# adam-kerrigan/pybader

Measured on AMD Instinct MI355X. Metric: Mvoxels/s neargrid assign+refine on 512^3 grid, higher is better.
Workload: dtype f64; 1 GPU; 512^3 synthetic 8-Gaussian-atom cubic cell (BASELINE config 3), neargrid assign + neargrid edge refinement changed:2, density resident in HBM; method=neargrid, device_driven_slab_step=False, basins=8

## Files before the change

include/bader_hip.h:

```cpp
#ifndef BADER_HIP_H
#define BADER_HIP_H

#include <stdint.h>

#ifdef __cplusplus
extern "C" {
#endif

typedef struct xb_ctx xb_ctx;

enum { XB_OK = 0, XB_E_ARG = -1, XB_E_HIP = -2, XB_E_STATE = -3, XB_E_LIMIT = -4, XB_E_COMM = -5,
       XB_E_SHORT = -6  };

enum { XB_I8 = 1, XB_I16 = 2, XB_I32 = 4, XB_I64 = 8 };

enum { XB_METHOD_ONGRID = 0, XB_METHOD_NEARGRID = 1 };
enum { XB_REFINE_ALL = 0, XB_REFINE_CHANGED = 1 };

const char *xb_last_error(void);
int xb_device_count(void);
int xb_create(int device, xb_ctx **out);
void xb_destroy(xb_ctx *c);
int xb_sync(xb_ctx *c);
void *xb_stream(xb_ctx *c);
// ... 188 lines not shown
enum {
    XB_REGIONS_BOXES = 1,
    XB_REGIONS_BRICKS = 2
};
enum { XB_DROP_TABLE_AND_MAXIMA = 2 };
enum {
    XB_CHECK_NO_MIRROR = 1,
    XB_CHECK_GENERIC_WALKER = 2,
    XB_CHECK_FULL_TGRAD = 4,
    XB_CHECK_LIST_DILATE = 8,
    XB_CHECK_WIDE_HALO = 16,
    XB_CHECK_NO_EC_SHARE = 32,
    XB_CHECK_IO_GATHER = 64
};
#define XB_CHECK_BRICK_LOOKUP 128
enum {
    XB_DBG_EC_PASSES = 4,
    XB_DBG_SLAB_STATS = 16,
    XB_DBG_STAGE_WAIT = 32,
    XB_DBG_SHORT_TIERS = 64
};
int xb_set_option(xb_ctx *c, int key, int value);
int xb_host_alloc(int64_t bytes, void **out);
int xb_host_free(void *p);
int xb_memory_stats(xb_ctx *c, int64_t *bytes_total, int64_t *bytes_table, int64_t *bytes_scratch);
int xb_box_stats(xb_ctx *c, int64_t *n_boxes, int64_t *box_voxels);
int xb_brick_labels(xb_ctx *c, int32_t *out, int64_t capacity, int64_t dims[3]);
int xb_slow_path_stats(xb_ctx *c, int64_t *assign_total, int64_t *refine_total);
int xb_deferred_stats(xb_ctx *c, int64_t *refine_total);
int xb_growth_stats(xb_ctx *c, int64_t *retries, int64_t *kill_launches);

int xb_comm_unique_id(uint8_t id_out[128]);
int xb_comm_init(xb_ctx *c, int rank, int nranks, const uint8_t id_in[128]);
int xb_comm_destroy(xb_ctx *c);
int xb_comm_exchange_planes(xb_ctx *c, int which, int n_send, const int32_t *send_peer, const int64_t *send_xa,
                            const int64_t *send_xb, int n_recv, const int32_t *recv_peer, const int64_t *recv_xa,
                            const int64_t *recv_xb);
int xb_comm_allreduce_i64(xb_ctx *c, int64_t *inout, int64_t n, int op);
int xb_comm_allgather_i64(xb_ctx *c, const int64_t *in, int64_t n, int64_t *out);
int xb_comm_share_brick_masks(xb_ctx *c, const int64_t *first, const int64_t *count);
int xb_comm_allgather_block(xb_ctx *c, int which, const int64_t *first, const int64_t *count);
int xb_comm_allreduce_block(xb_ctx *c);
int xb_comm_info(xb_ctx *c, int64_t out[4]);
int xb_comm_stats(xb_ctx *c, int64_t *bytes_sent);
// ... 6 lines not shown
```

pybader_amd/_lib.py:

```python
import ctypes as C
import threading
import os

import numpy as np

HERE = os.path.dirname(os.path.abspath(__file__))
LIB_PATH = os.environ.get('XB_LIBRARY') or os.path.join(HERE, 'libbader_hip.so')

METHODS = {'ongrid': 0, 'neargrid': 1}
REFINE_MODES = {'all': 0, 'changed': 1}
DTYPE_CODE = {np.dtype(np.int8): 1, np.dtype(np.int16): 2, np.dtype(np.int32): 4, np.dtype(np.int64): 8}
(XB_XC_EDGES, XB_XC_CHANGED, XB_XC_ESCAPED, XB_XC_TRAVELLING, XB_XC_SLOW, XB_XC_LOST, XB_XC_MINE, XB_XC_ROUNDS,
 XB_XC_COUNT) = range(9)
(XB_TIMER_ASSIGN, XB_TIMER_OG_MASKS, XB_TIMER_EDGE_FIND, XB_TIMER_REFINE_TRACE, XB_TIMER_MASKS_GROWTH, XB_TIMER_BRICK_MASKS,
 XB_TIMER_TRACE, XB_TIMER_BRICK_RECORDS, XB_TIMER_MOMENTS, XB_TIMER_ADJACENCY, XB_TIMER_MERGE, XB_TIMER_COUNT) = range(12)
XB_OPT_REGIONS = 1
XB_REGIONS_BOXES, XB_REGIONS_BRICKS = 1, 2
XB_OPT_CROSS_CHECK = 2
(XB_CHECK_NO_MIRROR, XB_CHECK_GENERIC_WALKER, XB_CHECK_FULL_TGRAD, XB_CHECK_LIST_DILATE, XB_CHECK_WIDE_HALO,
 XB_CHECK_NO_EC_SHARE, XB_CHECK_IO_GATHER) = (1, 2, 4, 8, 16, 32, 64)
CROSS_CHECK_BRICK_LOOKUP = 128
XB_OPT_DEBUG = 3
XB_DBG_EC_PASSES, XB_DBG_SLAB_STATS, XB_DBG_STAGE_WAIT, XB_DBG_SHORT_TIERS = 4, 16, 32, 64
XB_OPT_EC_GROUPS = 4
XB_OPT_EC_QCAP = 5
XB_OPT_DROP_TABLE = 6
XB_DROP_TABLE_AND_MAXIMA = 2
XB_OPT_KILL_LAUNCHES = 17
XB_OPT_SELF_EXCHANGE = 19
XB_OPT_ASYNC_COMM = 24
XB_OPT_WEIGHT_NO_LABELS = 30
XB_VORONOI_FULL_SEARCH = 1
XB_VORONOI_CAND_MAX = 512
XB_CRITICAL_FLOOD = 1
(XB_CRITICAL_MAXIMA, XB_CRITICAL_BOND_VOXELS, XB_CRITICAL_BOND_SUM, XB_CRITICAL_RING_VOXELS, XB_CRITICAL_RING_SUM,
 XB_CRITICAL_MINIMA, XB_CRITICAL_COUNTS) = range(7)
# ... 108 lines not shown
    'xb_plane_elems': (_i64, [_vp]),
    'xb_copy_planes': (_int, [_vp, _int, _int, _vp, _i64, _i64]),
    'xb_label_wire': (_int, [_vp, _int, _vp]),
    'xb_host_alloc': (_int, [_i64, _vp]),
    'xb_host_free': (_int, [_vp]),
    'xb_brick_masks_copy': (_int, [_vp, _int, _vp, _i64, _i64]),
    'xb_set_halo': (_int, [_vp, _i64]),
    'xb_kernel_time': (_int, [_vp, _int, _pdbl, _pi64]),
    'xb_kernel_time_reset': (_int, [_vp]),
    'xb_enable_timing': (_int, [_vp, _int]),
    'xb_set_option': (_int, [_vp, _int, _int]),
    'xb_box_stats': (_int, [_vp, _pi64, _pi64]),
    'xb_brick_labels': (_int, [_vp, _vp, _i64, _pi64]),
    'xb_slow_path_stats': (_int, [_vp, _pi64, _pi64]),
    'xb_deferred_stats': (_int, [_vp, _pi64]),
    'xb_growth_stats': (_int, [_vp, _pi64, _pi64]),
    'xb_comm_unique_id': (_int, [_vp]),
    'xb_comm_init': (_int, [_vp, _int, _int, _vp]),
    'xb_comm_destroy': (_int, [_vp]),
    'xb_comm_exchange_planes': (_int, [_vp, _int, _int, _vp, _pi64, _pi64, _int, _vp, _pi64, _pi64]),
    'xb_comm_allreduce_i64': (_int, [_vp, _pi64, C.c_int64, _int]),
    'xb_comm_allgather_i64': (_int, [_vp, _pi64, C.c_int64, _pi64]),
    'xb_comm_share_brick_masks': (_int, [_vp, _pi64, _pi64]),
    'xb_comm_allgather_block': (_int, [_vp, _int, _pi64, _pi64]),
    'xb_comm_allreduce_block': (_int, [_vp]),
    'xb_slab_supported': (_int, [_vp, _int, _pi64]),
    'xb_slab_assign_masks': (_int, [_vp, _int, _int]),
    'xb_slab_assign_trace': (_int, [_vp]),
    'xb_slab_assign_finish': (_int, [_vp, _pi64, _pi64]),
    'xb_slab_refine_pass': (_int, [_vp]),
# ... 906 lines not shown
    def slow_path_stats(self):
        a, b = C.c_int64(), C.c_int64()
        check(self.lib.xb_slow_path_stats(self.h, C.byref(a), C.byref(b)))
        return a.value, b.value

    def growth_stats(self):
        a, b = C.c_int64(), C.c_int64()
        check(self.lib.xb_growth_stats(self.h, C.byref(a), C.byref(b)))
        return a.value, b.value

    def deferred_stats(self):
        a = C.c_int64()
        check(self.lib.xb_deferred_stats(self.h, C.byref(a)))
        return a.value

    def sync(self):
        check(self.lib.xb_sync(self.h))


def critical_lut():
    out = np.zeros(XB_CRITICAL_LUT_SIZE, np.uint8)
    check(load().xb_critical_lut(_ptr(out)))
    return out


def hirshfeld_images(lattice, atoms_cart, species, r_cut):
    lat, at = _f64(lattice).reshape(9), _f64(atoms_cart).reshape(-1, 3)
    sp, rc = np.ascontiguousarray(species, dtype=np.int32).reshape(-1), _f64(r_cut).reshape(-1)
    if sp.shape[0] != at.shape[0]:
        raise ValueError(f'hirshfeld_images: {sp.shape[0]} species for {at.shape[0]} atoms')
# ... 36 lines not shown
```

pybader_amd/csrc/bader_hip.hip:

```cpp
#include "bader_kernels.h"
#include "../../include/bader_hip.h"

#include <algorithm>
#include <cmath>
#include <cstdarg>
#include <cstdio>
#include <cstring>
#include <mutex>
#include <string>
#include <thread>
#include <vector>

static thread_local long long xb_waits = 0;
static inline hipError_t xb_counted_sync(hipStream_t s) { xb_waits++; return (hipStreamSynchronize)(s); }
#define hipStreamSynchronize(s) xb_counted_sync(s)

#include "k_common.h"
#include "k_masks.h"
#include "k_fused.h"
#include "k_trace.h"
#include "k_ongrid.h"
#include "k_edges.h"
#include "k_sums.h"
#include "k_text.h"
// ... 49 lines not shown
    long long ec_buf_cap = 0;
    double *dist_dev = nullptr;
    int *boxbuf = nullptr;
    int *box_max_tab = nullptr;
    int n_boxes = 0;
    long long box_voxels = 0;
    struct Options {
        int boxes = 1, bricks = 1;
        int mirror = 1;
        int lean = 1;
        int mask_diag = 1;
        int tile_dilate = 1;
        int narrow_halo = 1;
        int ec_share = 1;
        int nb_bits = 1;
        int io_tiled = 1;
        int dbg = 0;
        int ec_groups = 256;
        int ec_qcap = EC_Q;
        int self_exchange = 0;
        int async_comm = 0;
        bool weight_no_labels = false;
    } opt;
    int *ec_share = nullptr;
    std::vector<int64_t> esc_starts, esc_offsets, esc_vox;
    unsigned long long *ec_pend = nullptr;
    int8_t *ec_pflag = nullptr;
    std::vector<int8_t> esc_complete;
    bool has_vacuum = true;
    bool vac_by_tol = false;
// ... 7 lines not shown
    int *walk = nullptr;
    int table_margin = -1;
    bool table_prebuilt = false;
    int table_stage = 0;
    std::vector<int> window_seeds;
    bool window_ties = true;
    bool slab_sparse = false;
    int ec_local_n = 0;
    int walk_n_out = 0;
    void *walk_out_dev = nullptr;
    std::vector<int64_t> walk_host, res_host;
    int walk_n_res = 0;
    void *walk_in = nullptr, *walk_out2 = nullptr, *walk_res = nullptr;
    long long walk_cap = 0;
    long long stat_deferred = 0;
    long long stat_ovf_assign = 0, stat_ovf_refine = 0;
    int *bres_last = nullptr;
    int *blab = nullptr;
    int nbk[3] = {0, 0, 0};
    bool grad_valid = false;
    bool grad_nb = false;
    bool brick_max_valid = false;
    int grad_cover = 0;
    unsigned char *brick_rec = nullptr;
    unsigned long long *nb_tab = nullptr;
    void *xbuf = nullptr;
    int slab_rank = 0, slab_nranks = 0, slab_stage = 0;
    void *wbuf[2] = {nullptr, nullptr};
    void *wk_in = nullptr;
    int wbuf_ranks = 0, walk_last = -1, walk_round = 0, wcap = 0;
    int walk_send = 0;
    int grow_kill_launches = 6;
    long long stat_grow_retries = 0;
    bool defer_wait = false;
    bool pending_assign = false;
    int64_t pending_n_maxima = 0;
    int grad_rule = 0;
// ... 180 lines not shown
#include "host_weight.h"
#include "host_moments.h"
#include "host_adjacency.h"
#include "host_merge.h"
#include "host_voronoi.h"
#include "host_critical.h"
#include "host_stencil.h"
#include "host_hirshfeld.h"

int xb_set_option(xb_ctx *c, int key, int value) {
    if (!c) return fail(XB_E_ARG, "null ctx");
    bool ok = true;
    switch (key) {
    case XB_OPT_REGIONS: c->opt.boxes = (value & XB_REGIONS_BOXES) != 0; c->opt.bricks = (value & XB_REGIONS_BRICKS) != 0; break;
    case XB_OPT_CROSS_CHECK:
        if (!(ok = value >= 0 && value < 2 * XB_CHECK_BRICK_LOOKUP)) break;
        c->opt.mirror = !(value & XB_CHECK_NO_MIRROR);
        c->opt.lean = !(value & XB_CHECK_GENERIC_WALKER);
        c->opt.mask_diag = !(value & XB_CHECK_FULL_TGRAD);
        c->opt.tile_dilate = !(value & XB_CHECK_LIST_DILATE);
        c->opt.narrow_halo = !(value & XB_CHECK_WIDE_HALO);
        c->opt.ec_share = !(value & XB_CHECK_NO_EC_SHARE);
        c->opt.io_tiled = !(value & XB_CHECK_IO_GATHER);
        c->opt.nb_bits = !(value & XB_CHECK_BRICK_LOOKUP);
        break;
    case XB_OPT_DEBUG: c->opt.dbg = value; break;
    case XB_OPT_EC_GROUPS: if ((ok = value >= 1 && value <= 4096)) c->opt.ec_groups = value; break;
    case XB_OPT_EC_QCAP: if ((ok = value >= 2 && value <= EC_Q)) c->opt.ec_qcap = value; break;
    case XB_OPT_DROP_TABLE: c->grad_valid = false; c->grad_nb = false; if (value == XB_DROP_TABLE_AND_MAXIMA) c->brick_max_valid = false; break;
    case XB_OPT_KILL_LAUNCHES: if ((ok = value >= 1)) c->grow_kill_launches = value; break;
    case XB_OPT_SELF_EXCHANGE: c->opt.self_exchange = value != 0; break;
    case XB_OPT_ASYNC_COMM: c->opt.async_comm = value != 0; break;
    case XB_OPT_WEIGHT_NO_LABELS: c->opt.weight_no_labels = value != 0; break;
    default: ok = false;
    }
    if (!ok) return fail(XB_E_ARG, "xb_set_option: unknown key %d", key);
    return XB_OK;
}
int xb_growth_stats(xb_ctx *c, int64_t *retries, int64_t *kill_launches) {
    if (!c) return fail(XB_E_ARG, "null ctx");
    if (retries) *retries = c->stat_grow_retries;
    if (kill_launches) *kill_launches = c->grow_kill_launches;
    return XB_OK;
}
int xb_deferred_stats(xb_ctx *c, int64_t *refine_total) {
    if (!c) return fail(XB_E_ARG, "null ctx");
    if (refine_total) *refine_total = c->stat_deferred;
    return XB_OK;
}
int xb_slow_path_stats(xb_ctx *c, int64_t *assign_total, int64_t *refine_total) {
    if (!c) return fail(XB_E_ARG, "null ctx");
    if (assign_total) *assign_total = c->stat_ovf_assign;
    if (refine_total) *refine_total = c->stat_ovf_refine;
    return XB_OK;
}
int xb_memory_stats(xb_ctx *c, int64_t *bytes_total, int64_t *bytes_table, int64_t *bytes_scratch) {
    if (!c || !c->has_grid) return fail(XB_E_STATE, "xb_memory_stats: no grid");
    const long long N = c->N;
    const long long table = c->grad_cap * (long long)sizeof(GradRec);
    const long long scratch = c->list_cap * 4 + (long long)c->stage_bytes + c->ec_buf_cap * 4 + (c->ec_pend ? 8 * N + 16 : 0) +
                              (c->w_cap ? 25 * c->w_cap + (c->w_S ? 8 * c->w_cap : 0) : 0)  +
                              (long long)c->m_cap * 8  +
// ... 94 lines not shown
```

pybader_amd/csrc/host_assign.h:

```cpp

static GridL light(const Grid &g);

static int ensure_brick_bytes(xb_ctx *c, int nbr) {
    if (c->blab_alloc < nbr) {
        hipFree(c->blab_buf); c->blab_buf = nullptr; c->blab_alloc = 0; c->brick_rec = nullptr; c->nb_tab = nullptr; c->brick_max_valid = false;
        if (c->grad_cover) { c->grad_cover = 0; c->grad_valid = false; c->grad_nb = false; }
        const size_t rec_bytes = ((size_t)nbr + 16 + 7) & ~(size_t)7;
        HIPCHK(hipMalloc(&c->blab_buf, (size_t)nbr * sizeof(int) + rec_bytes + (size_t)nbr * sizeof(unsigned long long)));
        c->blab_alloc = nbr;
        c->brick_rec = reinterpret_cast<unsigned char *>(c->blab_buf + nbr);
        c->nb_tab = reinterpret_cast<unsigned long long *>(c->brick_rec + rec_bytes);
    }
    return XB_OK;
}

static int ensure_grad(xb_ctx *c, bool force, bool boxes, bool main_rule) {
    if (int rc = need_grad(c)) return rc;
    c->g.main_ties = main_rule ? 1 : 0;
    if (c->grad_valid && !force && (c->grad_rule == 2 || c->grad_rule == (main_rule ? 1 : 0))) return XB_OK;
    const Grid &g = c->g;
    if (c->grad_valid && !force && !boxes && c->grad_cover == 1 && c->brick_rec) {
        const int nb1r = (g.ny + BRK - 1) / BRK, nb2r = (g.nz + BRK - 1) / BRK, nbr = ((g.nx + BRK - 1) / BRK) * nb1r * nb2r;
        ScopedTimer t(c, XB_TIMER_MASKS_GROWTH);
        launch_brick_records(c, nullptr, nullptr, nbr, nb1r, nb2r);
// ... 2 lines not shown
        return XB_OK;
    }
    if (!force && !boxes && !table_windowed(c) && g.x0 == 0 && g.x1 == g.nx && g.nx >= 16 && g.ny >= 16 && g.nz >= 16) {
        const int nb0 = (g.nx + BRK - 1) / BRK, nb1 = (g.ny + BRK - 1) / BRK, nb2 = (g.nz + BRK - 1) / BRK, nbr = nb0 * nb1 * nb2;
        if (int rc = ensure_brick_bytes(c, nbr)) return rc;
        ScopedTimer t(c, XB_TIMER_MASKS_GROWTH);
        int *buni = reinterpret_cast<int *>(c->st);
        if (!c->buni_valid) k_label_uniform_list<<<4096, TPB, 0, c->stream>>>(light(g), c->labels, nb1, nb2, nullptr, nbr, nullptr, nullptr, buni, 0, nbr);
        c->buni_valid = true;
        k_buni3<<<(nbr + 255) / 256, 256, 0, c->stream>>>(nb0, nb1, nb2, buni, buni + nbr);
        k_flag_mixed_bricks<<<(nbr + 255) / 256, 256, 0, c->stream>>>(nbr, buni + nbr, c->brick_rec);
        launch_brick_records(c, nullptr, nullptr, nbr, nb1, nb2);
        HIPCHK(hipGetLastError());
        c->grad_valid = true;
        c->grad_cover = 1;
        c->grad_rule = main_rule ? 1 : 0;
        c->regions_labels = false;
        c->blab = nullptr;
        c->table_stage = 0;
        return XB_OK;
    }
    {
        const int nb0 = (g.nx + BRK - 1) / BRK, nb1 = (g.ny + BRK - 1) / BRK, nb2 = (g.nz + BRK - 1) / BRK, nbr = nb0 * nb1 * nb2;
        if (int rc = ensure_brick_bytes(c, nbr)) return rc;
        ScopedTimer t(c, XB_TIMER_MASKS_GROWTH);
        ScopedTimer t_masks(c, XB_TIMER_BRICK_MASKS);
        const int wb0 = table_windowed(c) ? g.wx0 / BRK : 0, wnb = table_windowed(c) ? g.wlen / BRK : nb0;
        k_flag_window_bricks<<<(nbr + 255) / 256, 256, 0, c->stream>>>(nb0, nb1 * nb2, wb0, wnb, (unsigned char)3, c->brick_rec);
        launch_brick_records(c, nullptr, nullptr, nbr, nb1, nb2);
        HIPCHK(hipGetLastError());
    }
    c->grad_valid = true;
    c->grad_cover = 1;
    c->grad_rule = main_rule ? 1 : 0;
    c->window_ties = true;
    c->n_boxes = 0;
    c->box_voxels = 0;
    c->blab = nullptr;
    c->regions_labels = false;
    c->window_seeds.clear();
    c->table_stage = 2;
    (void)boxes;
    return XB_OK;
}

static int upload_pinned(xb_ctx *c, void *dst, const void *src, size_t bytes, size_t slot = 0) {
    if (!bytes) return XB_OK;
    if (slot + bytes > c->pin_bytes) {
// ... 542 lines not shown
            if (part) k_og_masks<GridS, true><<<grid, TPB, 0, c->stream>>>(gs, c->rho, c->labels, small, 0, bmask, bmaxv, bpot);
            else k_og_masks<GridS, false><<<grid, TPB, 0, c->stream>>>(gs, c->rho, c->labels, small, 0, bmask, bmaxv, bpot);
        } else {
            if (part) k_og_masks<Grid, true><<<grid, TPB, 0, c->stream>>>(g, c->rho, c->labels, small, 0, bmask, bmaxv, bpot);
            else k_og_masks<Grid, false><<<grid, TPB, 0, c->stream>>>(g, c->rho, c->labels, small, 0, bmask, bmaxv, bpot);
        }
    }
    {
        ScopedTimer t_growth(c, XB_TIMER_MASKS_GROWTH);
        launch_region_growth(c, nb0, nb1, nb2, bmask, bmaxv, bpot, seed, buf0, buf1, box_max, box_first, true);
        HIPCHK(hipGetLastError());
    }
    c->grad_valid = false; c->grad_nb = false;
    c->grad_cover = 0;
    c->brick_max_valid = true;
    c->blab = c->blab_buf;
    c->regions_neargrid = false;
    c->walk = walk;
    c->bres_last = nullptr;
    c->nbk[0] = nb0; c->nbk[1] = nb1; c->nbk[2] = nb2;
    {
        ScopedTimer t_assign(c, XB_TIMER_ASSIGN);
        int bits = 0;
        while ((1 << bits) < std::max(std::max(nb0, nb1), nb2)) bits++;
        const unsigned n_codes = 1u << (3 * bits);
        k_brick_walk_list_morton<<<(n_codes + 16 * TPB - 1) / (16 * TPB), TPB, 0, c->stream>>>(nb0, nb1, nb2, n_codes, c->blab, walk,
                                                                                              fs + FS_N_WALK, fs + FS_GROW_RETRY);
        k_note_regions<<<1, XB_BOXES_MAX, 0, c->stream>>>(gl, nb1, nb2, fs, box_first, box_max, c->first, c->max_list, fs + FS_N_MAX, c->max_cap);
        c->regions_pending = true;
        k_og_walk_dev<<<16384, XB_WAVE, 0, c->stream>>>(gl, box_max, c->blab, nb1, nb2, walk, fs, c->labels, c->first, c->max_list, c->max_cap,
// ... 79 lines not shown
```

pybader_amd/csrc/host_refine.h:

```cpp

static void plane_range(const Grid &g, int ext, int &xa, int &np) {
    const int own = g.x1 - g.x0;
    if (own + 2 * ext >= g.nx) { xa = 0; np = g.nx; }
    else { xa = ((g.x0 - ext) % g.nx + g.nx) % g.nx; np = own + 2 * ext; }
}

static int preset_known_planes(xb_ctx *c, int p0, int np) {
    const Grid &g = c->g;
    const int run1 = std::min(np, g.nx - p0);
    HIPCHK(hipMemsetAsync(c->known + (size_t)p0 * g.nyz, 2, (size_t)run1 * g.nyz, c->stream));
    if (np > run1) HIPCHK(hipMemsetAsync(c->known, 2, (size_t)(np - run1) * g.nyz, c->stream));
    return XB_OK;
}
static int *launch_brick_uniformity(xb_ctx *c, const GridL &gl, int b_off, int count, unsigned scan_grid) {
    const Grid &g = c->g;
    const int nb0 = (g.nx + 7) / 8, nb1 = (g.ny + 7) / 8, nb2 = (g.nz + 7) / 8, nbr = nb0 * nb1 * nb2;
    int *buni = reinterpret_cast<int *>(c->st);
    if (!c->buni_valid)
        k_label_uniform_list<<<scan_grid, TPB, 0, c->stream>>>(gl, c->labels, nb1, nb2, nullptr, count, nullptr, nullptr, buni, b_off, nbr);
    k_buni3<<<(nbr + 255) / 256, 256, 0, c->stream>>>(nb0, nb1, nb2, buni, buni + nbr);
    return buni + nbr;
}

static int edge_find_launch(xb_ctx *c, bool *dilate_owned) {
    const Grid &g = c->g;
    const bool whole = (g.x1 - g.x0 == g.nx);
    if (!whole && c->halo < 2) return fail(XB_E_STATE, "xb_edge_find: slab needs a label halo (xb_set_halo)");
    int xa, np, xb_, npd;
    const bool all = whole || (g.x1 - g.x0) + 2 * c->halo >= g.nx;
    plane_range(g, all ? g.nx : c->halo - 1, xa, np);
    plane_range(g, all ? g.nx : c->halo - 2, xb_, npd);
    HIPCHK(hipMemsetAsync(c->counters + CT_N_EDGES, 0, sizeof(int), c->stream));
    {
        ScopedTimer t(c, XB_TIMER_EDGE_FIND);
        const GridL gl = light(g);
        const int small = small_grid(g);
        int *buni = nullptr;
        if ((g.nx % 8 == 0 && g.ny % 8 == 0 && g.nz % 8 == 0) || (whole && g.nx >= 16 && g.ny >= 16 && g.nz >= 16)) {
            const int per_plane = ((g.ny + 7) / 8) * ((g.nz + 7) / 8);
            int b_off = 0, count = ((g.nx + 7) / 8) * per_plane;
            if (!all && np + 32 < g.nx) {
                const int p0 = ((xa - 8) % g.nx + g.nx) % g.nx;
                b_off = (p0 / 8) * per_plane;
                count = ((np + 8 + 7 + (p0 % 8)) / 8 + 1) * per_plane;
            }
            if (!c->buni_valid) c->buni_halo_safe = false;
            buni = launch_brick_uniformity(c, gl, b_off, count, (unsigned)std::min(4096, (count + 3) / 4));
        }
        const GradRec *G = c->grad_valid ? c->grad : nullptr;
        const unsigned char *brec = c->grad_valid && c->grad_cover == 1 ? c->brick_rec : nullptr;
        if (whole || all) {
            dim3 grid((g.nz + ET_Z - 1) / ET_Z, (g.ny + ET_Y - 1) / ET_Y, (np + ET_X - 1) / ET_X);
            k_edge_flag_tiled<<<grid, TPB, 0, c->stream>>>(gl, c->rho, c->labels, c->known, xa, np, c->list,
                                                           c->counters + CT_N_EDGES, small, buni, G, brec, c->has_vacuum ? 0 : 1);
            if (!whole)
                k_edge_dilate<<<nblocks((long long)npd * g.nyz), TPB, 0, c->stream>>>(g, c->known, xb_, npd, -2);
        } else if (buni && g.x0 % ET_X == 0 && g.x1 % ET_X == 0 && g.ny % ET_Y == 0 &&
                   (g.x1 - g.x0) + 2 * ((c->halo - 1 + ET_X - 1) / ET_X * ET_X) <= g.nx) {
            const int own = g.x1 - g.x0, side4 = (c->halo - 1 + ET_X - 1) / ET_X * ET_X;
            const int nty = g.ny / ET_Y, ntz = (g.nz + ET_Z - 1) / ET_Z;
            const int left0 = ((g.x0 - side4) % g.nx + g.nx) % g.nx, right0 = g.x1 % g.nx;
            if (int rc = preset_known_planes(c, left0, side4 + own + side4)) return rc;
            const int n_own = (own / ET_X) * nty * ntz, n_halo = 2 * (side4 / ET_X) * nty * ntz;
            int *tiles_own = (int *)c->stage, *tiles_halo = tiles_own + n_own, *halo_list = tiles_halo + n_halo;
            HIPCHK(hipMemsetAsync(c->counters + CT_HALO_EDGES, 0, sizeof(int), c->stream));
// ... 526 lines not shown

int xb_prepare_refine(xb_ctx *c) {
    NEED_GRID("xb_prepare_refine");
    return ensure_grad(c, false, false, false);
}

#define XB_STEP_REDO 1000
static int refine_iteration_fused(xb_ctx *c, int64_t *edges, int64_t *changed, bool late_records = false) {
    const Grid &g = c->g;
    int *fs = c->fs;
    c->g.main_ties = 0;
    const GridL gl = light(g);
    static_assert(FS_N_CHGLIST == FS_N_EDGES + 6, "one memset clears the refinement's counters");
    HIPCHK(hipMemsetAsync(fs + FS_N_EDGES, 0, 7 * sizeof(int), c->stream));
    c->chg_n = -1;
    {
        ScopedTimer t(c, XB_TIMER_EDGE_FIND);
        const int small = small_grid(g);
        int *buni = nullptr;
        int ntiles_listed = 0;
        if (g.nx >= 16 && g.ny >= 16 && g.nz >= 16)
            buni = launch_brick_uniformity(c, gl, 0, ((g.nx + 7) / 8) * ((g.ny + 7) / 8) * ((g.nz + 7) / 8), 4096);
        const unsigned char *brec = (c->grad_valid && c->grad_cover == 1) || late_records ? c->brick_rec : nullptr;
        if (buni) {
            const int ntiles = ((g.nz + ET_Z - 1) / ET_Z) * ((g.ny + ET_Y - 1) / ET_Y) * ((g.nx + ET_X - 1) / ET_X);
            ntiles_listed = ntiles;
            int *tiles = (int *)c->stage;
            HIPCHK(hipMemsetAsync(c->known, 2, (size_t)c->N, c->stream));
            k_edge_tile_list<<<(ntiles + TPB - 1) / TPB, TPB, 0, c->stream>>>(gl, buni, tiles, fs + FS_N_TILES, 0, (g.nx + ET_X - 1) / ET_X,
                                                                              c->pending_assign ? fs : nullptr);
            k_edge_flag_listed<<<std::min(ntiles, 2048), TPB, 0, c->stream>>>(gl, c->rho, c->labels, c->known, c->list, fs + FS_N_EDGES, small,
                                                           c->grad_valid ? c->grad : nullptr, brec, c->has_vacuum ? 0 : 1, tiles, fs + FS_N_TILES);
        } else {
            dim3 grid((g.nz + ET_Z - 1) / ET_Z, (g.ny + ET_Y - 1) / ET_Y, (g.nx + ET_X - 1) / ET_X);
            k_edge_flag_tiled<<<grid, TPB, 0, c->stream>>>(gl, c->rho, c->labels, c->known, 0, g.nx, c->list, fs + FS_N_EDGES, small, buni,
                                                           c->grad_valid ? c->grad : nullptr, brec, c->has_vacuum ? 0 : 1);
        }
        if (buni && c->opt.tile_dilate && g.nz % ET_Z == 0) k_edge_dilate_tiles<<<std::min(ntiles_listed, 4096), TPB, 0, c->stream>>>(gl, c->known, (const int *)c->stage, fs + FS_N_TILES);
        else k_edge_dilate_list<<<nblocks(c->N / 16), TPB, 0, c->stream>>>(gl, c->known, c->list, 0, fs + FS_N_EDGES);
    }
    c->list_valid = false; c->chg_n = -1;
    c->buni_valid = false;
    if (late_records) {
        if (int rc = need_grad(c)) return rc;
        ScopedTimer t(c, XB_TIMER_MASKS_GROWTH);
        const int nb0 = (g.nx + 7) / 8, nb1 = (g.ny + 7) / 8, nb2 = (g.nz + 7) / 8, nbr = nb0 * nb1 * nb2;
        unsigned char *band = reinterpret_cast<unsigned char *>(c->blab_buf);
        HIPCHK(hipMemsetAsync(band, 0, (size_t)nbr, c->stream));
        k_flag_band_bricks<<<4096, TPB, 0, c->stream>>>(gl, c->known, (const int *)c->stage, fs + FS_N_TILES, band);
        k_rec_set_bit0<<<(nbr + 255) / 256, 256, 0, c->stream>>>(nbr, c->brick_rec, band);
        launch_brick_records(c, nullptr, nullptr, nbr, nb1, nb2);
        HIPCHK(hipGetLastError());
        c->grad_valid = true;
        c->grad_cover = 1;
        c->grad_rule = 0;
// ... 156 lines not shown
```

pybader_amd/csrc/host_stages.h:

```cpp

enum { BB_TOTAL = 1 << 20, BB_REGMAX = 1 << 16, BB_REGFIRST = 1 << 17 };

static bool table_windowed(const xb_ctx *c) { return c->g.wlen < c->g.nx; }
static int small_grid(const Grid &g) { return g.nx < 16 || g.ny < 16 || g.nz < 80; }
static int trace_maxsteps(const Grid &g) { return 8 * (g.nx + g.ny + g.nz) + 64; }
static const int *slab_regions_of(const xb_ctx *c) {
    const Grid &g = c->g;
    return (table_windowed(c) && c->blab && c->regions_labels && !c->has_vacuum && (c->grad_rule == 2 || c->slab_sparse) &&
            g.nx % 8 == 0 && g.ny % 8 == 0 && g.nz % 8 == 0) ? c->blab : nullptr;
}

static_assert(CT_REDO == CT_N_MAX + 15, "a host-driven assignment zeroes CT_N_MAX .. CT_REDO at once");
static int begin_assignment(xb_ctx *c, int *counts, int n, bool invalidate) {
    HIPCHK(hipMemsetAsync(counts, 0, n * sizeof(int), c->stream));
    if (!c->first_clean) {
        k_fill<int><<<4096, TPB, 0, c->stream>>>(c->first, XB_INT_MAX, c->N);
        HIPCHK(hipGetLastError());
    }
    c->first_clean = false;
    c->regions_pending = false;
    if (invalidate) {
        c->buni_valid = false; c->regions_labels = false;
        c->list_valid = false; c->chg_n = -1;
    }
// ... 3 lines not shown
static void launch_brick_masks(xb_ctx *c, bool part, bool allow_diag, int *bmask, int *bmaxv, int *bpot) {
    const Grid &g = c->g;
    const dim3 grid((g.nz + GT_Z - 1) / GT_Z, (g.ny + GT_Y - 1) / GT_Y, (g.x1 - g.x0 + GT_X - 1) / GT_X);
    GridS gs;
    const bool sym = sym_grid(g, gs);
    int mirror = 0;
    double mu_scale = 0.;
    if (sym && c->opt.mirror) mirror_prefilter(g, mirror, mu_scale);
    const bool diag = allow_diag && c->opt.mask_diag && g.T[1] == 0. && g.T[2] == 0. && g.T[3] == 0. && g.T[5] == 0. && g.T[6] == 0. && g.T[7] == 0.;
    auto launch = [&](auto kernel, const auto &gt) {
        kernel<<<grid, TPB, 0, c->stream>>>(gt, c->rho, small_grid(g), bmask, bmaxv, c->fs + FS_TIES, g.x0, mu_scale, mirror, bpot);
    };
    if (!sym) launch(part ? k_brick_masks<Grid, 1, false, true> : k_brick_masks<Grid, 1, false>, g);
    else if (part) launch(diag ? k_brick_masks<GridS, 1, true, true> : k_brick_masks<GridS, 1, false, true>, gs);
    else launch(diag ? k_brick_masks<GridS, 1, true> : k_brick_masks<GridS, 1, false>, gs);
}

static bool nb_bits_ok(const xb_ctx *c) { return c->grad_valid && c->grad_nb && c->opt.nb_bits; }
static void launch_brick_records(xb_ctx *c, const int *list, const int *n_dev, int nbr, int nb1, int nb2) {
    const Grid &g = c->g;
    const bool part = g.nx % BRK || g.ny % BRK || g.nz % BRK;
    const bool mark = !table_windowed(c) && g.x0 == 0 && g.x1 == g.nx && !part && (!list || c->blab) && c->nb_tab;
    c->grad_nb = mark;
    if (mark)
        k_nb_table<<<(nbr + 255) / 256, 256, 0, c->stream>>>(nbr / (nb1 * nb2), nb1, nb2, list ? c->blab : nullptr, c->brick_rec, c->nb_tab);
    auto launch = [&](auto kernel, const auto &gt) {
        kernel<<<4096, TPB, 0, c->stream>>>(gt, c->rho, c->grad, list, n_dev, nbr, nb1, nb2, c->brick_rec, small_grid(g),
                                            mark ? c->nb_tab : nullptr);
    };
    GridS gs;
// ... 97 lines not shown
```

pybader_amd/csrc/k_edges.h:

```cpp
#pragma once

__device__ __forceinline__ void classify27(const Grid &g, const double *__restrict__ rho,
                                           const int *__restrict__ labels, int x, int y, int z, int v,
                                           bool &is_edge, bool &is_max) {
    const int vol_num = labels[v];
    is_edge = false;
    is_max = true;
    int nb[27];
    int k = 0;
#pragma unroll
    for (int ix = -1; ix < 2; ix++) {
        const int tx = wrapi(x + ix, g.nx);
#pragma unroll
        for (int iy = -1; iy < 2; iy++) {
            const int ty = wrapi(y + iy, g.ny);
#pragma unroll
            for (int iz = -1; iz < 2; iz++) {
                const int tz = wrapi(z + iz, g.nz);
                const int l = lin3(g, tx, ty, tz);
                const int nv = labels[l];
                nb[k++] = (nv == -1) ? -1 : l;
                if (nv != -1 && nv != vol_num) is_edge = true;
            }
        }
// ... 418 lines not shown
    for (int item = part0 + blockIdx.x / n_xcd; item < part1; item += gridDim.x / n_xcd) {
        const unsigned entry = (unsigned)tiles[item];
        const int t = (int)(entry & 0x7fffffffu);
        const int tx0 = (t / (ntz * nty)) * ET_X, y0 = ((t / ntz) % nty) * ET_Y, z0 = (t % ntz) * ET_Z;
        if (entry & 0x80000000u) {
            for (int i = threadIdx.x; i < ET_X * ET_Y * ET_Z; i += TPB) {
                const int z = z0 + (i % ET_Z), y = y0 + (i / ET_Z) % ET_Y, x = tx0 + i / (ET_Z * ET_Y);
                if (z < g.nz && y < g.ny && x < g.nx) known[(x * g.ny + y) * g.nz + z] = 0;
            }
            continue;
        }
        __syncthreads();
        int salt = 0;
        asm volatile("" : "+v"(salt));
        edge_tile(g, rho, labels, known, 0, g.nx, list, list_count, small, nullptr, G, brick_rec, no_vacuum, tx0, y0, z0, salt);
    }
}

__global__ __launch_bounds__(TPB) void k_list_changed(const int *__restrict__ list, const int *n_dev, const int8_t *__restrict__ known,
                                                      int *__restrict__ out, int *out_count, int out_cap, const int *n_changed) {
    __shared__ int s_buf[BlockAppender<1>::CAP], s_n[2];
    if (*n_changed == 0) return;
    BlockAppender<1> app;
    app.init(s_buf, s_n, out, out_count, out_cap);
    const int n = *n_dev;
    for (int base = blockIdx.x * TPB; base < n; base += gridDim.x * TPB) {
        const int t = base + threadIdx.x;
        const int v = t < n ? list[t] : 0;
        const bool hit = t < n && known[v] == -2;
        app.add(hit ? 1 : 0, [&](int) { return v; });
// ... 800 lines not shown
```

Baseline: 43480 Mvoxels/s.

## Add wave-ballot bitmask edge sweep fusing edge flag and dilation

Adds a new edge-finding kernel that loads a haloed label tile into shared memory and builds per-row 64-bit equality masks with wave ballots. Edge, near-edge and dilation status are then derived with bitwise shifts instead of a per-voxel 27-neighbour scan. Maxima exclusion is checked only for candidate voxels in maxima-flagged bricks. Edge detection and dilation become one launch, which removes a separate dilation pass and most redundant label reads. The path is gated by grid divisibility, no vacuum, few maxima, and not being right after blanket brick records, so it adds complexity and a fallback path.

Result: faster. 44330 Mvoxels/s (median of 6 runs) (+2.0%).

```diff
diff --git a/include/bader_hip.h b/include/bader_hip.h
--- a/include/bader_hip.h
+++ b/include/bader_hip.h
@@ -226,6 +226,7 @@
     XB_CHECK_IO_GATHER = 64
 };
 #define XB_CHECK_BRICK_LOOKUP 128
+#define XB_CHECK_VOXEL_SWEEP 256
 enum {
     XB_DBG_EC_PASSES = 4,
     XB_DBG_SLAB_STATS = 16,
@@ -240,6 +241,7 @@
 int xb_brick_labels(xb_ctx *c, int32_t *out, int64_t capacity, int64_t dims[3]);
 int xb_slow_path_stats(xb_ctx *c, int64_t *assign_total, int64_t *refine_total);
 int xb_deferred_stats(xb_ctx *c, int64_t *refine_total);
+int xb_sweep_stats(xb_ctx *c, int64_t *bit_sweeps, int64_t *voxel_sweeps);
 int xb_growth_stats(xb_ctx *c, int64_t *retries, int64_t *kill_launches);
 
 int xb_comm_unique_id(uint8_t id_out[128]);
diff --git a/pybader_amd/_lib.py b/pybader_amd/_lib.py
--- a/pybader_amd/_lib.py
+++ b/pybader_amd/_lib.py
@@ -20,6 +20,7 @@
 (XB_CHECK_NO_MIRROR, XB_CHECK_GENERIC_WALKER, XB_CHECK_FULL_TGRAD, XB_CHECK_LIST_DILATE, XB_CHECK_WIDE_HALO,
  XB_CHECK_NO_EC_SHARE, XB_CHECK_IO_GATHER) = (1, 2, 4, 8, 16, 32, 64)
 CROSS_CHECK_BRICK_LOOKUP = 128
+CROSS_CHECK_VOXEL_SWEEP = 256
 XB_OPT_DEBUG = 3
 XB_DBG_EC_PASSES, XB_DBG_SLAB_STATS, XB_DBG_STAGE_WAIT, XB_DBG_SHORT_TIERS = 4, 16, 32, 64
 XB_OPT_EC_GROUPS = 4
@@ -158,6 +159,7 @@
     'xb_brick_labels': (_int, [_vp, _vp, _i64, _pi64]),
     'xb_slow_path_stats': (_int, [_vp, _pi64, _pi64]),
     'xb_deferred_stats': (_int, [_vp, _pi64]),
+    'xb_sweep_stats': (_int, [_vp, _pi64, _pi64]),
     'xb_growth_stats': (_int, [_vp, _pi64, _pi64]),
     'xb_comm_unique_id': (_int, [_vp]),
     'xb_comm_init': (_int, [_vp, _int, _int, _vp]),
@@ -1094,6 +1096,11 @@
         check(self.lib.xb_deferred_stats(self.h, C.byref(a)))
         return a.value
 
+    def sweep_stats(self):
+        a, b = C.c_int64(), C.c_int64()
+        check(self.lib.xb_sweep_stats(self.h, C.byref(a), C.byref(b)))
+        return a.value, b.value
+
     def sync(self):
         check(self.lib.xb_sync(self.h))
 
diff --git a/pybader_amd/csrc/bader_hip.hip b/pybader_amd/csrc/bader_hip.hip
--- a/pybader_amd/csrc/bader_hip.hip
+++ b/pybader_amd/csrc/bader_hip.hip
@@ -87,6 +87,7 @@
         int narrow_halo = 1;
         int ec_share = 1;
         int nb_bits = 1;
+        int bit_sweep = 1;
         int io_tiled = 1;
         int dbg = 0;
         int ec_groups = 256;
@@ -124,6 +125,7 @@
     void *walk_in = nullptr, *walk_out2 = nullptr, *walk_res = nullptr;
     long long walk_cap = 0;
     long long stat_deferred = 0;
+    long long stat_bit_sweeps = 0, stat_voxel_sweeps = 0;
     long long stat_ovf_assign = 0, stat_ovf_refine = 0;
     int *bres_last = nullptr;
     int *blab = nullptr;
@@ -131,6 +133,7 @@
     bool grad_valid = false;
     bool grad_nb = false;
     bool brick_max_valid = false;
+    bool brick_max_blanket = false;
     int grad_cover = 0;
     unsigned char *brick_rec = nullptr;
     unsigned long long *nb_tab = nullptr;
@@ -341,7 +344,7 @@
     switch (key) {
     case XB_OPT_REGIONS: c->opt.boxes = (value & XB_REGIONS_BOXES) != 0; c->opt.bricks = (value & XB_REGIONS_BRICKS) != 0; break;
     case XB_OPT_CROSS_CHECK:
-        if (!(ok = value >= 0 && value < 2 * XB_CHECK_BRICK_LOOKUP)) break;
+        if (!(ok = value >= 0 && value < 2 * XB_CHECK_VOXEL_SWEEP)) break;
         c->opt.mirror = !(value & XB_CHECK_NO_MIRROR);
         c->opt.lean = !(value & XB_CHECK_GENERIC_WALKER);
         c->opt.mask_diag = !(value & XB_CHECK_FULL_TGRAD);
@@ -350,6 +353,7 @@
         c->opt.ec_share = !(value & XB_CHECK_NO_EC_SHARE);
         c->opt.io_tiled = !(value & XB_CHECK_IO_GATHER);
         c->opt.nb_bits = !(value & XB_CHECK_BRICK_LOOKUP);
+        c->opt.bit_sweep = !(value & XB_CHECK_VOXEL_SWEEP);
         break;
     case XB_OPT_DEBUG: c->opt.dbg = value; break;
     case XB_OPT_EC_GROUPS: if ((ok = value >= 1 && value <= 4096)) c->opt.ec_groups = value; break;
@@ -373,6 +377,12 @@
 int xb_deferred_stats(xb_ctx *c, int64_t *refine_total) {
     if (!c) return fail(XB_E_ARG, "null ctx");
     if (refine_total) *refine_total = c->stat_deferred;
+    return XB_OK;
+}
+int xb_sweep_stats(xb_ctx *c, int64_t *bit_sweeps, int64_t *voxel_sweeps) {
+    if (!c) return fail(XB_E_ARG, "null ctx");
+    if (bit_sweeps) *bit_sweeps = c->stat_bit_sweeps;
+    if (voxel_sweeps) *voxel_sweeps = c->stat_voxel_sweeps;
     return XB_OK;
 }
 int xb_slow_path_stats(xb_ctx *c, int64_t *assign_total, int64_t *refine_total) {
diff --git a/pybader_amd/csrc/host_assign.h b/pybader_amd/csrc/host_assign.h
--- a/pybader_amd/csrc/host_assign.h
+++ b/pybader_amd/csrc/host_assign.h
@@ -40,6 +40,7 @@
         HIPCHK(hipGetLastError());
         c->grad_valid = true;
         c->grad_cover = 1;
+        c->brick_max_blanket = true;
         c->grad_rule = main_rule ? 1 : 0;
         c->regions_labels = false;
         c->blab = nullptr;
@@ -58,6 +59,7 @@
     }
     c->grad_valid = true;
     c->grad_cover = 1;
+    c->brick_max_blanket = true;
     c->grad_rule = main_rule ? 1 : 0;
     c->window_ties = true;
     c->n_boxes = 0;
@@ -630,6 +632,7 @@
     c->grad_valid = false; c->grad_nb = false;
     c->grad_cover = 0;
     c->brick_max_valid = true;
+    c->brick_max_blanket = false;
     c->blab = c->blab_buf;
     c->regions_neargrid = false;
     c->walk = walk;
diff --git a/pybader_amd/csrc/host_refine.h b/pybader_amd/csrc/host_refine.h
--- a/pybader_amd/csrc/host_refine.h
+++ b/pybader_amd/csrc/host_refine.h
@@ -20,6 +20,20 @@
         k_label_uniform_list<<<scan_grid, TPB, 0, c->stream>>>(gl, c->labels, nb1, nb2, nullptr, count, nullptr, nullptr, buni, b_off, nbr);
     k_buni3<<<(nbr + 255) / 256, 256, 0, c->stream>>>(nb0, nb1, nb2, buni, buni + nbr);
     return buni + nbr;
+}
+
+static bool sweep_bits_ok(const xb_ctx *c, const int *buni) {
+    const Grid &g = c->g;
+    if (c->grad_valid && c->grad_cover == 1 && c->brick_max_blanket) return false;
+    const long long nbr = (long long)((g.nx + 7) / 8) * ((g.ny + 7) / 8) * ((g.nz + 7) / 8);
+    if (8 * (long long)c->maxima_sorted.size() >= nbr) return false;
+    return c->opt.bit_sweep && c->opt.tile_dilate && buni && !c->has_vacuum && g.x0 == 0 && g.x1 == g.nx && g.nx % ET_X == 0 &&
+           g.ny % ET_Y == 0 && g.nz % ET_Z == 0 && !small_grid(g);
+}
+static void launch_sweep_bits(xb_ctx *c, const GridL &gl, int ntiles, int *edge_count, const GradRec *G, const unsigned char *brec,
+                              const int *tiles, const int *n_tiles) {
+    k_edge_sweep_bits<<<std::min(ntiles, 2048), TPB, 0, c->stream>>>(gl, c->rho, c->labels, c->known, c->list, edge_count, G, brec, tiles, n_tiles);
+    c->stat_bit_sweeps++;
 }
 
 static int edge_find_launch(xb_ctx *c, bool *dilate_owned) {
@@ -49,6 +63,18 @@
         }
         const GradRec *G = c->grad_valid ? c->grad : nullptr;
         const unsigned char *brec = c->grad_valid && c->grad_cover == 1 ? c->brick_rec : nullptr;
+        if (whole && sweep_bits_ok(c, buni)) {
+            const int ntiles = (g.nz / ET_Z) * (g.ny / ET_Y) * (g.nx / ET_X);
+            int *tiles = (int *)c->stage;
+            HIPCHK(hipMemsetAsync(c->known, 2, (size_t)c->N, c->stream));
+            HIPCHK(hipMemsetAsync(c->counters + CT_TILES_OWN, 0, sizeof(int), c->stream));
+            k_edge_tile_list<<<(ntiles + TPB - 1) / TPB, TPB, 0, c->stream>>>(gl, buni, tiles, c->counters + CT_TILES_OWN, 0, g.nx / ET_X);
+            launch_sweep_bits(c, gl, ntiles, c->counters + CT_N_EDGES, G, brec, tiles, c->counters + CT_TILES_OWN);
+            HIPCHK(hipGetLastError());
+            *dilate_owned = false;
+            return XB_OK;
+        }
+        c->stat_voxel_sweeps++;
         if (whole || all) {
             dim3 grid((g.nz + ET_Z - 1) / ET_Z, (g.ny + ET_Y - 1) / ET_Y, (np + ET_X - 1) / ET_X);
             k_edge_flag_tiled<<<grid, TPB, 0, c->stream>>>(gl, c->rho, c->labels, c->known, xa, np, c->list,
@@ -605,6 +631,7 @@
     static_assert(FS_N_CHGLIST == FS_N_EDGES + 6, "one memset clears the refinement's counters");
     HIPCHK(hipMemsetAsync(fs + FS_N_EDGES, 0, 7 * sizeof(int), c->stream));
     c->chg_n = -1;
+    bool bits = false;
     {
         ScopedTimer t(c, XB_TIMER_EDGE_FIND);
         const int small = small_grid(g);
@@ -620,16 +647,22 @@
             HIPCHK(hipMemsetAsync(c->known, 2, (size_t)c->N, c->stream));
             k_edge_tile_list<<<(ntiles + TPB - 1) / TPB, TPB, 0, c->stream>>>(gl, buni, tiles, fs + FS_N_TILES, 0, (g.nx + ET_X - 1) / ET_X,
                                                                               c->pending_assign ? fs : nullptr);
-            k_edge_flag_listed<<<std::min(ntiles, 2048), TPB, 0, c->stream>>>(gl, c->rho, c->labels, c->known, c->list, fs + FS_N_EDGES, small,
-                                                           c->grad_valid ? c->grad : nullptr, brec, c->has_vacuum ? 0 : 1, tiles, fs + FS_N_TILES);
+            if ((bits = sweep_bits_ok(c, buni)))
+                launch_sweep_bits(c, gl, ntiles, fs + FS_N_EDGES, c->grad_valid ? c->grad : nullptr, brec, tiles, fs + FS_N_TILES);
+            else
+                k_edge_flag_listed<<<std::min(ntiles, 2048), TPB, 0, c->stream>>>(gl, c->rho, c->labels, c->known, c->list, fs + FS_N_EDGES, small,
+                                                               c->grad_valid ? c->grad : nullptr, brec, c->has_vacuum ? 0 : 1, tiles, fs + FS_N_TILES);
         } else {
             dim3 grid((g.nz + ET_Z - 1) / ET_Z, (g.ny + ET_Y - 1) / ET_Y, (g.nx + ET_X - 1) / ET_X);
             k_edge_flag_tiled<<<grid, TPB, 0, c->stream>>>(gl, c->rho, c->labels, c->known, 0, g.nx, c->list, fs + FS_N_EDGES, small, buni,
                                                            c->grad_valid ? c->grad : nullptr, brec, c->has_vacuum ? 0 : 1);
         }
-        if (buni && c->opt.tile_dilate && g.nz % ET_Z == 0) k_edge_dilate_tiles<<<std::min(ntiles_listed, 4096), TPB, 0, c->stream>>>(gl, c->known, (const int *)c->stage, fs + FS_N_TILES);
-        else k_edge_dilate_list<<<nblocks(c->N / 16), TPB, 0, c->stream>>>(gl, c->known, c->list, 0, fs + FS_N_EDGES);
-    }
+        if (!bits) {
+            if (buni && c->opt.tile_dilate && g.nz % ET_Z == 0) k_edge_dilate_tiles<<<std::min(ntiles_listed, 4096), TPB, 0, c->stream>>>(gl, c->known, (const int *)c->stage, fs + FS_N_TILES);
+            else k_edge_dilate_list<<<nblocks(c->N / 16), TPB, 0, c->stream>>>(gl, c->known, c->list, 0, fs + FS_N_EDGES);
+        }
+    }
+    if (!bits) c->stat_voxel_sweeps++;
     c->list_valid = false; c->chg_n = -1;
     c->buni_valid = false;
     if (late_records) {
diff --git a/pybader_amd/csrc/host_stages.h b/pybader_amd/csrc/host_stages.h
--- a/pybader_amd/csrc/host_stages.h
+++ b/pybader_amd/csrc/host_stages.h
@@ -41,6 +41,7 @@
     if (!sym) launch(part ? k_brick_masks<Grid, 1, false, true> : k_brick_masks<Grid, 1, false>, g);
     else if (part) launch(diag ? k_brick_masks<GridS, 1, true, true> : k_brick_masks<GridS, 1, false, true>, gs);
     else launch(diag ? k_brick_masks<GridS, 1, true> : k_brick_masks<GridS, 1, false>, gs);
+    c->brick_max_blanket = false;
 }
 
 static bool nb_bits_ok(const xb_ctx *c) { return c->grad_valid && c->grad_nb && c->opt.nb_bits; }
diff --git a/pybader_amd/csrc/k_edges.h b/pybader_amd/csrc/k_edges.h
--- a/pybader_amd/csrc/k_edges.h
+++ b/pybader_amd/csrc/k_edges.h
@@ -456,6 +456,264 @@
         int salt = 0;
         asm volatile("" : "+v"(salt));
         edge_tile(g, rho, labels, known, 0, g.nx, list, list_count, small, nullptr, G, brick_rec, no_vacuum, tx0, y0, z0, salt);
+    }
+}
+
+#define EB_X (ET_X + 4)
+#define EB_Y (ET_Y + 4)
+#define EB_P (ET_Z + 4)
+#define EB_ROWS (EB_X * EB_Y)
+#define EB_RING ((ET_X + 2) * (ET_Y + 2))
+typedef unsigned long long eb_mask;
+__device__ __forceinline__ eb_mask eb_ballot(bool b) { return __builtin_amdgcn_ballot_w64(b); }
+__device__ __forceinline__ void eb_park(unsigned &lo, unsigned &hi, eb_mask m, bool here) {
+    lo = here ? (unsigned)m : lo;
+    hi = here ? (unsigned)(m >> 32) : hi;
+}
+__device__ __forceinline__ unsigned eb_eq4(const int4 &a, const int4 &b) {
+    return (a.x == b.x ? 1u : 0u) | (a.y == b.y ? 2u : 0u) | (a.z == b.z ? 4u : 0u) | (a.w == b.w ? 8u : 0u);
+}
+__device__ __forceinline__ bool eb_is_max(const GridL &g, const double *__restrict__ rho, int x, int y, int z) {
+    const int v = (x * g.ny + y) * g.nz + z;
+    const double c = rho[v];
+    bool is_max = true;
+#pragma unroll 1
+    for (int dx = -1; dx < 2; dx++) {
+        const int X = wrapi(x + dx, g.nx);
+#pragma unroll 1
+        for (int dy = -1; dy < 2; dy++) {
+            const int Y = wrapi(y + dy, g.ny);
+#pragma unroll
+            for (int dz = -1; dz < 2; dz++)
+                if (rho[(X * g.ny + Y) * g.nz + wrapi(z + dz, g.nz)] > c) is_max = false;
+        }
+    }
+    return is_max;
+}
+__global__ __launch_bounds__(TPB) void k_edge_sweep_bits(GridL g, const double *__restrict__ rho, const int *__restrict__ labels,
+                                                         int8_t *__restrict__ known, int *__restrict__ list, int *list_count,
+                                                         const GradRec *__restrict__ G, const unsigned char *__restrict__ brick_rec,
+                                                         const int *__restrict__ tiles, const int *n_tiles) {
+    static_assert(ET_Z == XB_WAVE && TPB == 4 * XB_WAVE && EB_X == 8 && EB_ROWS == 4 * 24 && ET_X == 4 && ET_Y == 8, "tile shape");
+    __shared__ __attribute__((aligned(16))) int tile[EB_ROWS][EB_P];
+    __shared__ eb_mask sP[EB_ROWS], sCx[EB_ROWS], sE[ET_X * ET_Y], sNear[ET_X * ET_Y];
+    __shared__ unsigned sHi[EB_ROWS];
+    __shared__ int sOff[ET_X * ET_Y];
+    __shared__ eb_mask sQ[2], sRE[EB_RING], sRC[EB_RING];
+    __shared__ unsigned sREh[EB_RING], sRCh[EB_RING];
+    __shared__ unsigned char sB[ET_X + 2][3][12];
+    const int n = *n_tiles;
+    const int ntz = g.nz / ET_Z, nty = g.ny / ET_Y, nb1 = g.ny >> 3, nb2 = g.nz >> 3;
+    const int n_xcd = (gridDim.x % 8 == 0) ? 8 : 1;
+    const int part = (n + n_xcd - 1) / n_xcd, part0 = (int)(blockIdx.x % n_xcd) * part, part1 = min(n, part0 + part);
+#pragma unroll 1
+    for (int item = part0 + blockIdx.x / n_xcd; item < part1; item += gridDim.x / n_xcd) {
+        int salt = 0;
+        asm volatile("" : "+v"(salt));
+        const int tid = (int)threadIdx.x + salt, lane = tid % XB_WAVE, wv = __builtin_amdgcn_readfirstlane(tid / XB_WAVE);
+        const unsigned entry = (unsigned)tiles[item];
+        const int t = (int)(entry & 0x7fffffffu);
+        const int tx0 = (t / (ntz * nty)) * ET_X, y0 = ((t / ntz) % nty) * ET_Y, z0 = (t % ntz) * ET_Z;
+        if (entry & 0x80000000u) {
+            for (int i = tid; i < ET_X * ET_Y * ET_Z; i += TPB)
+                known[((size_t)(tx0 + i / (ET_Z * ET_Y)) * g.ny + y0 + (i / ET_Z) % ET_Y) * g.nz + z0 + i % ET_Z] = 0;
+            continue;
+        }
+        int a[24];
+        {
+            int yoff[EB_Y];
+#pragma unroll
+            for (int ey = 0; ey < EB_Y; ey++) yoff[ey] = wrap_u(y0 - 2 + ey, g.ny) * g.nz + z0;
+#pragma unroll
+            for (int e = 0; e < 2; e++) {
+                const int *plane = labels + (size_t)wrap_u(tx0 - 2 + 2 * wv + e, g.nx) * g.nyz;
+#pragma unroll
+                for (int ey = 0; ey < EB_Y; ey++) a[e * EB_Y + ey] = plane[yoff[ey] + lane];
+            }
+            int hv[2] = {0, 0};
+#pragma unroll
+            for (int k = 0; k < 2; k++) {
+                const int i = tid + k * TPB;
+                if (i < 4 * EB_ROWS) {
+                    const int row = i >> 2, q = i & 3;
+                    const int X = wrap_u(tx0 - 2 + row / EB_Y, g.nx), Y = wrap_u(y0 - 2 + row % EB_Y, g.ny);
+                    const int Z = wrap_u(q < 2 ? z0 + ET_Z + q : z0 - 4 + q, g.nz);
+                    hv[k] = labels[((size_t)X * g.ny + Y) * g.nz + Z];
+                }
+            }
+            int bv = 3;
+            const int bi = tid - (TPB - (ET_X + 2) * 30);
+            if (bi >= 0 && brick_rec) {
+                const int X = wrap_u(tx0 - 1 + bi / 30, g.nx);
+                bv = brick_rec[((X >> 3) * nb1 + wrap_u((y0 >> 3) - 1 + (bi / 10) % 3, nb1)) * nb2 + wrap_u((z0 >> 3) - 1 + bi % 10, nb2)];
+            }
+#pragma unroll
+            for (int j = 0; j < 24; j++) tile[24 * wv + j][lane] = a[j];
+#pragma unroll
+            for (int k = 0; k < 2; k++) {
+                const int i = tid + k * TPB;
+                if (i < 4 * EB_ROWS) tile[i >> 2][ET_Z + (i & 3)] = hv[k];
+            }
+            if (bi >= 0) sB[bi / 30][(bi / 10) % 3][bi % 10] = (unsigned char)bv;
+        }
+        __syncthreads();
+        {
+            unsigned ql = 0, qh = 0, xl = 0, xh = 0;
+#pragma unroll
+            for (int e = 0; e < 2; e++) {
+                const int r0 = 24 * wv + EB_Y * e;
+                int b[EB_Y], nx[EB_Y];
+#pragma unroll
+                for (int ey = 0; ey < EB_Y; ey++) b[ey] = tile[r0 + ey][lane + 1];
+                if (e == 1) {
+#pragma unroll
+                    for (int ey = 0; ey < EB_Y; ey++) nx[ey] = tile[min(r0 + EB_Y + ey, EB_ROWS - 1)][lane];
+                }
+                eb_mask zm = 0, zc = eb_ballot(a[EB_Y * e] == b[0]), ym = 0;
+#pragma unroll
+                for (int ey = 0; ey < EB_Y; ey++) {
+                    const int j = EB_Y * e + ey;
+                    const eb_mask zp = ey + 1 < EB_Y ? eb_ballot(a[j + 1] == b[ey + 1]) : 0ull;
+                    const eb_mask yc = ey + 1 < EB_Y ? eb_ballot(a[j] == a[j + 1]) : 0ull;
+                    const eb_mask cx = eb_ballot(a[j] == (e == 0 ? a[j + EB_Y] : nx[ey]));
+                    const bool here = lane == j;
+                    eb_park(ql, qh, zm & zc & zp & ym & yc, here);
+                    eb_park(xl, xh, cx, here);
+                    zm = zc; zc = zp; ym = yc;
+                    asm volatile("" : "+v"(ql), "+v"(qh), "+v"(xl), "+v"(xh));
+                }
+            }
+            const eb_mask Q = ((eb_mask)qh << 32) | ql, Cx = ((eb_mask)xh << 32) | xl;
+            const int r = min(24 * wv + lane, EB_ROWS - 1);
+            const int4 h = *reinterpret_cast<const int4 *>(&tile[r][ET_Z]);
+            const int4 hy = *reinterpret_cast<const int4 *>(&tile[min(r + 1, EB_ROWS - 1)][ET_Z]);
+            const int4 hx = *reinterpret_cast<const int4 *>(&tile[min(r + EB_Y, EB_ROWS - 1)][ET_Z]);
+            const int first = tile[r][0];
+            const unsigned Zh = (h.x == h.y ? 1u : 0u) | (h.y == h.z ? 2u : 0u) | (h.z == h.w ? 4u : 0u) | (h.w == first ? 8u : 0u);
+            const unsigned Cyh = (r % EB_Y != EB_Y - 1) ? eb_eq4(h, hy) : 0u, Cxh = (r + EB_Y < EB_ROWS) ? eb_eq4(h, hx) : 0u;
+            const unsigned pk = Zh | (Cyh << 4);
+            const unsigned pkm = __shfl_up(pk, 1), pkp = __shfl_down(pk, 1);
+            const unsigned Qh = pkm & pk & pkp & (pkm >> 4) & (pk >> 4) & 15u;
+            if (lane < 24) {
+                sP[r] = Q & ((Q << 1) | (Qh >> 3));
+                sCx[r] = Cx;
+                sHi[r] = (Qh & ((Qh << 1) | (unsigned)(Q >> 63)) & 15u) | (Cxh << 4);
+            }
+        }
+        __syncthreads();
+        const bool ring = lane < EB_RING;
+        const int rl = min(lane, EB_RING - 1), rx = rl / (ET_Y + 2), ry = rl % (ET_Y + 2);
+        eb_mask E = 0;
+        unsigned Eh = 0;
+        auto finish = [&]() {
+            const eb_mask D = E | (E << 1) | (E >> 1) | (eb_mask)((Eh >> 3) & 1u) | ((eb_mask)(Eh & 1u) << 63);
+            const eb_mask Dy = __shfl_up(D, 1) | D | __shfl_down(D, 1);
+            const eb_mask Dn = __shfl_up(Dy, ET_Y + 2) | Dy | __shfl_down(Dy, ET_Y + 2);
+            const bool own = ring && rx >= 1 && rx <= ET_X && ry >= 1 && ry <= ET_Y;
+            const int cnt = own ? __popcll(E) : 0;
+            int incl = cnt;
+#pragma unroll
+            for (int o = 1; o < XB_WAVE; o <<= 1) {
+                const int up = __shfl_up(incl, o);
+                if (lane >= o) incl += up;
+            }
+            const int total = __shfl(incl, XB_WAVE - 1);
+            int base = 0;
+            if (total) {
+                if (lane == 0) base = atomicAdd(list_count, total);
+                base = __shfl(base, 0);
+            }
+            if (own) {
+                const int row = (rx - 1) * ET_Y + ry - 1;
+                sE[row] = E; sNear[row] = Dn; sOff[row] = base + incl - cnt;
+            }
+        };
+        if (wv == 0) {
+            const int r = (rx + 1) * EB_Y + ry + 1;
+            const unsigned hm = sHi[r - EB_Y], h0 = sHi[r], hp = sHi[r + EB_Y];
+            E = ring ? ~(sP[r - EB_Y] & sP[r] & sP[r + EB_Y] & sCx[r - EB_Y] & sCx[r]) : 0ull;
+            Eh = ring ? ~(hm & h0 & hp & (hm >> 4) & (h0 >> 4)) & 9u : 0u;
+            const unsigned char *bb = sB[rx][ry == 0 ? 0 : (ry == ET_Y + 1 ? 2 : 1)];
+            eb_mask F = 0;
+#pragma unroll
+            for (int k = 0; k < 8; k++)
+                if (bb[k + 1] & 2) F |= 0xFFull << (8 * k);
+            const unsigned Fh = ((bb[9] >> 1) & 1u) | (((bb[0] >> 1) & 1u) << 3);
+            const eb_mask qa = eb_ballot((E & F) != 0), qb = eb_ballot((Eh & Fh) != 0);
+            if (lane == 0) { sQ[0] = qa; sQ[1] = qb; }
+            if (qa | qb) {
+                if (ring) { sRE[lane] = E; sREh[lane] = Eh; sRC[lane] = E & F; sRCh[lane] = Eh & Fh; }
+            } else
+                finish();
+        }
+        __syncthreads();
+        if (sQ[0] | sQ[1]) {
+            eb_mask qa = sQ[0] & (0x1111111111111111ull << wv);
+            qa = ((eb_mask)(unsigned)__builtin_amdgcn_readfirstlane((int)(qa >> 32)) << 32) | (unsigned)__builtin_amdgcn_readfirstlane((int)qa);
+            if (wv == 3 && sQ[1]) {
+                const unsigned ch = ring ? sRCh[rl] : 0u;
+                const unsigned char *sb = sB[rx][ry == 0 ? 0 : (ry == ET_Y + 1 ? 2 : 1)];
+                const int X = wrap_u(tx0 - 1 + rx, g.nx), Y = wrap_u(y0 - 1 + ry, g.ny);
+                int Z[2], kw[2];
+                bool act[2], usek[2];
+#pragma unroll
+                for (int i = 0; i < 2; i++) {
+                    Z[i] = wrap_u(i == 0 ? z0 + ET_Z : z0 - 1, g.nz);
+                    act[i] = (ch >> (3 * i)) & 1u;
+                    usek[i] = G && act[i] && (sb[i == 0 ? 9 : 0] & 1) && plane_in_window(g, X);
+                    const int slot = usek[i] ? rec_slot(g, (X * g.ny + Y) * g.nz + Z[i]) : 0;
+                    kw[i] = G ? reinterpret_cast<const int *>(G)[(size_t)(unsigned)slot * 8 + 6] : 0;
+                }
+                unsigned clear = 0;
+#pragma unroll
+                for (int i = 0; i < 2; i++) {
+                    bool m = act[i] && !(usek[i] && low_og(kw[i] & 0x1FFFFF) != XB_OG_SELF);
+                    if (m) m = eb_is_max(g, rho, X, Y, Z[i]);
+                    if (m) clear |= 1u << (3 * i);
+                }
+                if (clear) sREh[rl] &= ~clear;
+            }
+            while (qa) {
+                int src[8], X[8], Y[8], kw[8];
+                bool act[8], usek[8];
+#pragma unroll
+                for (int i = 0; i < 8; i++) {
+                    src[i] = -1;
+                    if (qa) { src[i] = __ffsll((long long)qa) - 1; qa &= qa - 1; }
+                    const int sr = max(src[i], 0), sx = sr / (ET_Y + 2), sy = sr % (ET_Y + 2);
+                    const eb_mask c = sRC[sr];
+                    const unsigned char *sb = sB[sx][sy == 0 ? 0 : (sy == ET_Y + 1 ? 2 : 1)];
+                    X[i] = wrap_u(tx0 - 1 + sx, g.nx); Y[i] = wrap_u(y0 - 1 + sy, g.ny);
+                    act[i] = src[i] >= 0 && ((c >> lane) & 1ull);
+                    usek[i] = G && act[i] && (sb[1 + (lane >> 3)] & 1) && plane_in_window(g, X[i]);
+                    const int slot = usek[i] ? rec_slot(g, (X[i] * g.ny + Y[i]) * g.nz + z0 + lane) : 0;
+                    kw[i] = G ? reinterpret_cast<const int *>(G)[(size_t)(unsigned)slot * 8 + 6] : 0;
+                }
+#pragma unroll
+                for (int i = 0; i < 8; i++) {
+                    bool m = act[i] && !(usek[i] && low_og(kw[i] & 0x1FFFFF) != XB_OG_SELF);
+                    if (m) m = eb_is_max(g, rho, X[i], Y[i], z0 + lane);
+                    const eb_mask mm = eb_ballot(m);
+                    if (lane == 0 && src[i] >= 0 && mm) sRE[src[i]] &= ~mm;
+                }
+            }
+            __syncthreads();
+            if (wv == 0) {
+                E = ring ? sRE[rl] : 0ull;
+                Eh = ring ? sREh[rl] : 0u;
+                finish();
+            }
+            __syncthreads();
+        }
+#pragma unroll
+        for (int ty = 0; ty < ET_Y; ty++) {
+            const int row = wv * ET_Y + ty;
+            const eb_mask E = sE[row], N = sNear[row];
+            const int v = ((tx0 + wv) * g.ny + y0 + ty) * g.nz + z0 + lane;
+            const bool e = (E >> lane) & 1ull;
+            known[v] = e ? (int8_t)-2 : (((N >> lane) & 1ull) ? (int8_t)-1 : (int8_t)2);
+            if (e) list[sOff[row] + __popcll(E & ((1ull << lane) - 1ull))] = v;
+        }
     }
 }
 
```
